# zju3dv/BoxDreamer

Measured on AMD Instinct MI355X. Metric: poses/s/GPU (5-ref, 224×224, bf16); heatmap max-abs err vs CPU ref, higher is better.
Workload: dtype f16 + e4m3 corrections (BETR q, k columns: f16)

## Files before the change

### boxdreamer_amd/csrc/gemm_f16c8.hip

```cpp
#include "gemm_common.h"

#ifdef BD_GEMM_PROBE
extern "C" int bd_gemm_f16c8_probe_set(void* buf) {
    return (int)hipMemcpyToSymbol(HIP_SYMBOL(bd_probe_buf), &buf, sizeof(buf));
}
#endif

namespace {

template <int NSTAGE, int EP, int OUTK, bool GELU, int WM = 4, int WN = 2, int NPW = 4, bool LNF = false, bool SK = false>
__global__ __launch_bounds__((WM * WN + NPW) * 64, (WM * WN + NPW) <= 4 ? 2 : 1) void gemm_kernel_pc_f16c8(const bd_gemm_args p) {
    constexpr int MI = 2, NI = 3, NCW = WM * WN;
    constexpr int TBM = WM * MI * 32, TBN = WN * NI * 32, BK = 32;
    constexpr int A0 = TBM * 64, W0 = TBN * 64, A1 = TBM * 32, W1 = TBN * 64;
    constexpr int OFF_W0 = A0, OFF_A1 = A0 + W0, OFF_W1 = A0 + W0 + A1, STAGE = A0 + W0 + A1 + W1;
    constexpr int SR = 16, SCRATCH = NCW * SR * NI * 32 * 4, S2 = SCRATCH > STAGE ? SCRATCH : STAGE;
    static_assert(SCRATCH <= STAGE, "the epilogue scratch overlays stage 2");
    constexpr int GA0 = TBM / 16, GW0 = TBN / 16, GA1 = TBM / 32, GW1 = TBN / 16;
    constexpr int IA0 = (GA0 + NPW - 1) / NPW, IW0 = (GW0 + NPW - 1) / NPW, IA1 = (GA1 + NPW - 1) / NPW, IW1 = (GW1 + NPW - 1) / NPW;
    static_assert(GA0 % NPW == 0 && GW0 % NPW == 0 && GA1 % NPW == 0 && GW1 % NPW == 0, "every producer wave issues the same number of pieces (counted vmcnt)");
    constexpr int PIECES = IA0 + IW0 + IA1 + IW1;
    constexpr int WAIT_ONE_SLAB = (PIECES & 15) | ((PIECES >> 4) << 14) | 0x70 | 0xF00;
    constexpr int AUX_COLP = 2 * STAGE + S2, AUX_RMS = AUX_COLP + 4096, AUX_ROWS = AUX_RMS + 2048, AUX_BYTES = EP == 0 ? 0 : (LNF ? 10240 : 6144);
    static_assert(!LNF || (EP != 0 && NPW * 64 >= TBM && NSTAGE == 3), "LayerNorm fold: one producer lane per tile row");
    static_assert(!SK || ((EP == 3 || EP == 4 || EP == 5) && !LNF && NSTAGE == 3), "split-K: the fp32-residual epilogues, one tile per workgroup");
    __shared__ __attribute__((aligned(1024))) unsigned char lds[2 * STAGE + S2 + AUX_BYTES];

    bd_saturating_conversions();
    const int tid = threadIdx.x, lane = tid & 63;
    const int wid = __builtin_amdgcn_readfirstlane(tid >> 6);
    const int M = p.M, N = p.N;
    const int S = SK ? p.sk_split : 1;
    const int ks = SK ? ((int)blockIdx.x >> 3) % S : 0;
    const int nk_all = p.K / BK;
    const int k_lo = SK ? ks * nk_all / S : 0;
    const int nk = SK ? (ks + 1) * nk_all / S - k_lo : nk_all;
    const int tilesM = (M + TBM - 1) / TBM, tilesN = (N + TBN - 1) / TBN, nt = tilesM * tilesN;
    const int nwg = SK ? (int)gridDim.x / S : (int)gridDim.x;
    const int bid = SK ? ((int)blockIdx.x & 7) + 8 * (((int)blockIdx.x >> 3) / S) : (int)blockIdx.x, xcd = bid & 7;
    const int tq = nt >> 3, tr = nt & 7;
    const int t_begin = xcd < tr ? xcd * (tq + 1) : tr * (tq + 1) + (xcd - tr) * tq;
    const int t_end = t_begin + tq + (xcd < tr ? 1 : 0);
    const int stride = (nwg - xcd + 7) >> 3;
    constexpr int GROUP_M = 4;
    auto tile_origin = [&](int t, int& m0, int& n0) {
        const int per_group = GROUP_M * tilesN;
        const int g = t / per_group, in_g = t % per_group;
        const int gm0 = g * GROUP_M;
        const int gh = (tilesM - gm0) < GROUP_M ? (tilesM - gm0) : GROUP_M;
        m0 = (gm0 + in_g % gh) * TBM;
        n0 = (in_g / gh) * TBN;
    };
    const unsigned lds_off = lds_offset_of(lds);

    if (wid >= NCW) {
        const int pw = wid - NCW;
        const unsigned lda0 = (unsigned)(p.lda * 2), ldw0 = (unsigned)(p.ldw * 2), lda1 = (unsigned)p.lda, ldw1 = (unsigned)(p.ldw * 2);
        unsigned oA0[IA0], oW0[IW0], oA1[IA1], oW1[IW1];
#pragma unroll
        for (int i = 0; i < IA0; ++i) { const int row = (pw + NPW * i) * 16 + lane / 4; oA0[i] = row * lda0 + swz_chunk<4>(row, lane % 4) * 16; }
#pragma unroll
        for (int i = 0; i < IW0; ++i) { const int row = (pw + NPW * i) * 16 + lane / 4; oW0[i] = row * ldw0 + swz_chunk<4>(row, lane % 4) * 16; }
#pragma unroll
        for (int i = 0; i < IA1; ++i) { const int row = (pw + NPW * i) * 32 + lane / 2; oA1[i] = row * lda1 + swz_chunk<2>(row, lane % 2) * 16; }
#pragma unroll
        for (int i = 0; i < IW1; ++i) { const int row = (pw + NPW * i) * 16 + lane / 4; oW1[i] = row * ldw1 + swz_chunk<4>(row, lane % 4) * 16; }
        const unsigned char* pA0 = (const unsigned char*)p.A;
        const unsigned char* pW0 = (const unsigned char*)p.W;
        const unsigned char* pA1 = pA0 + p.a_plane * 2;
        const unsigned char* pW1 = pW0 + p.w_plane * 2;
        auto issue = [&](int stage, int m0, int n0, int kt) {
            const int rows_a = (M - m0) < TBM ? (M - m0) : TBM, rows_w = (N - n0) < TBN ? (N - n0) : TBN;
            const unsigned la0 = (unsigned)(rows_a - 1) * lda0 + 48, lw0 = (unsigned)(rows_w - 1) * ldw0 + 48;
            const unsigned la1 = (unsigned)(rows_a - 1) * lda1 + 16, lw1 = (unsigned)(rows_w - 1) * ldw1 + 48;
            const unsigned st = lds_off + stage * STAGE + pw * 1024;
            const unsigned char* ba0 = pA0 + (int64_t)m0 * lda0 + (int64_t)(k_lo + kt) * 64;
            const unsigned char* bw0 = pW0 + (int64_t)n0 * ldw0 + (int64_t)(k_lo + kt) * 64;
            const unsigned char* ba1 = pA1 + (int64_t)m0 * lda1 + (int64_t)(k_lo + kt) * 32;
            const unsigned char* bw1 = pW1 + (int64_t)n0 * ldw1 + (int64_t)(k_lo + kt) * 64;
#pragma unroll
            for (int i = 0; i < IA0; ++i) glds16_s(oA0[i] < la0 ? oA0[i] : la0, ba0, st + i * (NPW * 1024));
#pragma unroll
            for (int i = 0; i < IW0; ++i) glds16_s(oW0[i] < lw0 ? oW0[i] : lw0, bw0, st + OFF_W0 + i * (NPW * 1024));
#pragma unroll
            for (int i = 0; i < IA1; ++i) glds16_s(oA1[i] < la1 ? oA1[i] : la1, ba1, st + OFF_A1 + i * (NPW * 1024));
#pragma unroll
            for (int i = 0; i < IW1; ++i) glds16_s(oW1[i] < lw1 ? oW1[i] : lw1, bw1, st + OFF_W1 + i * (NPW * 1024));
        };
        int ig = 0, ist = 0, it = t_begin + (bid >> 3), ikt = 0, im0 = 0, in0 = 0, itn = 0;
        if (it < t_end) tile_origin(it, im0, in0);
        if constexpr (EP == 2) {
            if (pw == 1) {
                const unsigned off = (unsigned)lane * 16 < 368u ? (unsigned)lane * 16 : 368u;
                glds16_s(off, (const unsigned char*)p.rms_wq, lds_off + AUX_RMS);
                glds16_s(off, (const unsigned char*)p.rms_wk, lds_off + AUX_RMS + 1024);
            }
        }
        int lnt = 0;
        auto issue_next = [&]() {
            if (it >= t_end) return;
            if constexpr (EP != 0) {
                if (ikt == 0) {
                    if (pw == 0 && p.bias) {
                        const unsigned off = (unsigned)lane * 16 < (unsigned)(TBN * 4 - 16) ? (unsigned)lane * 16 : (unsigned)(TBN * 4 - 16);
                        glds16_s(off, (const unsigned char*)(p.bias + in0), lds_off + AUX_COLP + (itn & 1) * 2048);
                    }
                    if constexpr (LNF) {
                        if (pw == 1 % NPW) {
                            const unsigned off = (unsigned)lane * 16 < (unsigned)(TBN * 4 - 16) ? (unsigned)lane * 16 : (unsigned)(TBN * 4 - 16);
                            glds16_s(off, (const unsigned char*)(p.ln_colsum + in0), lds_off + AUX_COLP + (itn & 1) * 2048 + 1024);
                        }
                        if (pw * 64 + lane < TBM) {
                            int row = im0 + pw * 64 + lane;
                            row = row < M ? row : M - 1;
                            const f32x4* sp = (const f32x4*)(p.ln_stats_in + (int64_t)row * 16);
                            const f32x4 lnst[4] = {sp[0], sp[1], sp[2], sp[3]};
                            *(float2*)(lds + AUX_ROWS + (lnt & 1) * 2048 + (pw * 64 + lane) * 8) = ln_rows_combine(lnst, p.ln_eps);
                        }
                        ++lnt;
                        asm volatile("s_waitcnt lgkmcnt(0)" ::: "memory");
                    }
                    ++itn;
                }
            }
            issue(ist, im0, in0, ikt);
            ++ig;
            ist = ist + 1 == NSTAGE ? 0 : ist + 1;
            if (++ikt == nk) {
                ikt = 0;
                it += stride;
                if (it < t_end) tile_origin(it, im0, in0);
            }
        };
        auto wait_landed = [&](int slabs) {
            if (slabs <= 0) asm volatile("s_waitcnt vmcnt(0)" ::: "memory");
            else { __builtin_amdgcn_s_waitcnt(WAIT_ONE_SLAB); asm volatile("" ::: "memory"); }
        };
#ifdef BD_GEMM_PROBE
        unsigned probe_ts = 0;
#endif
#pragma unroll
        for (int i = 0; i < NSTAGE - 1; ++i) issue_next();
        int g = 0;
        for (int t = t_begin + (bid >> 3); t < t_end; t += stride) {
            for (int kt = 0; kt < nk; ++kt) {
                BD_PROBE_IF(g < 20, g * 3 + 2)
                wait_landed(ig - g - 1);
                BD_PROBE_IF(g < 20, g * 3)
                pc_barrier();
                BD_PROBE_IF(g < 20, g * 3 + 1)
                if (ig <= g + NSTAGE - 1) issue_next();
                ++g;
            }
            pc_barrier();
        }
#ifdef BD_GEMM_PROBE
        if (bd_probe_buf && blockIdx.x < 1024) bd_probe_buf[((size_t)blockIdx.x * 16 + wid) * 64 + lane] = probe_ts;
#endif
        return;
    }

    const int wm = wid / WN, wn = wid % WN;
    const int lrow = lane & 31, lhalf = lane >> 5;
    const int scale_a = 127, scale_w = 127 - (p.w_qexp + BD_F16C8_D);
    int g_st = 0;
#ifdef BD_GEMM_PROBE
    unsigned probe_ts = 0;
    int g = 0;
#endif
    BD_PROBE(58) BD_PROBE_RT(56)
    int ti = 0;
    f32x16 acc[MI][NI];
    const bool secondary = SK && ks != S - 1;
    if constexpr (EP != 0) {
        int m0, n0;
        tile_origin(t_begin + (bid >> 3), m0, n0);
        if (secondary) {
#pragma unroll
            for (int i = 0; i < MI; ++i)
#pragma unroll
                for (int j = 0; j < NI; ++j)
#pragma unroll
                    for (int r = 0; r < 16; ++r) acc[i][j][r] = 0.f;
        } else {
            acc_init<MI, NI>(p, acc, m0 + wm * (MI * 32), n0 + wn * (NI * 32), lane);
        }
    }
    for (int t = t_begin + (bid >> 3); t < t_end; t += stride, ++ti) {
        int m0, n0;
        tile_origin(t, m0, n0);
        if constexpr (EP == 0) acc_init<MI, NI>(p, acc, m0 + wm * (MI * 32), n0 + wn * (NI * 32), lane);
        for (int kt = 0; kt < nk; ++kt) {
            BD_PROBE_IF(g < 20, g * 3)
            pc_barrier();
            BD_PROBE_IF(g < 20, g * 3 + 1)
#ifdef BD_GEMM_PROBE
            ++g;
#endif
            const unsigned char* base = lds + g_st * STAGE;
            g_st = g_st + 1 == NSTAGE ? 0 : g_st + 1;
            f16x8 ah[2][MI], wh[2][NI];
            u128 al[MI];
            i32x8 w8[NI];
#define LD16(dst, ptr, row, ks) dst = __builtin_bit_cast(f16x8, *(const u128*)((ptr) + (row) * 64 + (swz_chunk<4>((row), (ks) * 2 + lhalf) << 4)));
#define LDLO(dst, ptr, row) dst = *(const u128*)((ptr) + (row) * 32 + (swz_chunk<2>((row), lhalf) << 4));
#define LDW8(dst, ptr, row)                                                                                    \
            {                                                                                                     \
                const u128 lo_ = *(const u128*)((ptr) + (row) * 64 + (swz_chunk<4>((row), 2 * lhalf) << 4));        \
                const u128 hi_ = *(const u128*)((ptr) + (row) * 64 + (swz_chunk<4>((row), 2 * lhalf + 1) << 4));    \
                dst = (i32x8){(int)lo_[0], (int)lo_[1], (int)lo_[2], (int)lo_[3], (int)hi_[0], (int)hi_[1], (int)hi_[2], (int)hi_[3]}; \
            }
#define Q8P(f, a, b) ((h2_){f[a], f[b]})
#define Q8H(d0, d1, f)                                                                                        \
            {                                                                                                     \
                typedef _Float16 h2_ __attribute__((ext_vector_type(2)));                                         \
                typedef short s2_ __attribute__((ext_vector_type(2)));                                            \
                s2_ a_ = {0, 0}, b_ = {0, 0};                                                                     \
                a_ = __builtin_amdgcn_cvt_scalef32_pk_fp8_f16(a_, Q8P(f, 0, 1), 1.0f, false);                     \
                a_ = __builtin_amdgcn_cvt_scalef32_pk_fp8_f16(a_, Q8P(f, 2, 3), 1.0f, true);                      \
                b_ = __builtin_amdgcn_cvt_scalef32_pk_fp8_f16(b_, Q8P(f, 4, 5), 1.0f, false);                     \
                b_ = __builtin_amdgcn_cvt_scalef32_pk_fp8_f16(b_, Q8P(f, 6, 7), 1.0f, true);                      \
                d0 = __builtin_bit_cast(unsigned, a_);                                                            \
                d1 = __builtin_bit_cast(unsigned, b_);                                                            \
            }
#pragma unroll
            for (int j = 0; j < NI; ++j) LD16(wh[0][j], base + OFF_W0, wn * (NI * 32) + j * 32 + lrow, 0)
#pragma unroll
            for (int i = 0; i < MI; ++i) LD16(ah[0][i], base, wm * (MI * 32) + i * 32 + lrow, 0)
            __builtin_amdgcn_sched_barrier(0);
            constexpr int NMM = MI * NI;
            static_assert(MI == 2 && NI == 3, "the interleave below is written for 2 x 3 MFMA tiles per wave");
            unsigned qd[MI][4];
#pragma unroll
            for (int q = 0; q < NMM; ++q) {
                const int i = q % MI, j = q / MI;
                acc[i][j] = __builtin_amdgcn_mfma_f32_32x32x16_f16(ah[0][i], wh[0][j], acc[i][j], 0, 0, 0);
                if (q < MI) LD16(ah[1][q], base, wm * (MI * 32) + q * 32 + lrow, 1)
                else if (q < MI + NI) LD16(wh[1][q - MI], base + OFF_W0, wn * (NI * 32) + (q - MI) * 32 + lrow, 1)
                if (q == 3) Q8H(qd[0][0], qd[0][1], ah[0][0])
                if (q == 4) Q8H(qd[1][0], qd[1][1], ah[0][1])
                __builtin_amdgcn_sched_barrier(0);
            }
#pragma unroll
            for (int q = 0; q < NMM; ++q) {
                const int i = q % MI, j = q / MI;
                acc[i][j] = __builtin_amdgcn_mfma_f32_32x32x16_f16(ah[1][i], wh[1][j], acc[i][j], 0, 0, 0);
                if (q < MI) LDLO(al[q], base + OFF_A1, wm * (MI * 32) + q * 32 + lrow)
                if (q == 2) LDW8(w8[0], base + OFF_W1, wn * (NI * 32) + lrow)
                if (q == 4) LDW8(w8[1], base + OFF_W1, wn * (NI * 32) + 32 + lrow)
                if (q == 2) Q8H(qd[0][2], qd[0][3], ah[1][0])
                if (q == 3) Q8H(qd[1][2], qd[1][3], ah[1][1])
                __builtin_amdgcn_sched_barrier(0);
            }
#pragma unroll
            for (int q = 0; q < NMM; ++q) {
                const int i = q % MI, j = q / MI;
                const i32x8 a8 = {(int)al[i][0], (int)al[i][1], (int)al[i][2], (int)al[i][3], (int)qd[i][0], (int)qd[i][1], (int)qd[i][2], (int)qd[i][3]};
                acc[i][j] = __builtin_amdgcn_mfma_scale_f32_32x32x64_f8f6f4(a8, w8[j], acc[i][j], 0, 0, 0, scale_a, 0, scale_w);
                if (q == 0) LDW8(w8[2], base + OFF_W1, wn * (NI * 32) + 64 + lrow)
                __builtin_amdgcn_sched_barrier(0);
            }
#undef LDW8
#undef LD16
#undef LDLO
#undef Q8H
#undef Q8P
        }
        BD_PROBE_IF(g == nk, 60)
        pc_barrier();
        BD_PROBE_IF(g == nk, 61)
        if constexpr (SK) {
            int* const flags = (int*)p.sk_ws;
            f32x4* const parts = (f32x4*)((unsigned char*)p.sk_ws + BD_SPLITK_FLAG_BYTES);
            if (secondary) {
                const int idx = (t * 3 + ks) * NCW + wid;
                f32x4* dst = parts + (size_t)idx * (MI * NI * 4 * 64) + lane;
#pragma unroll
                for (int i = 0; i < MI; ++i)
#pragma unroll
                    for (int j = 0; j < NI; ++j)
#pragma unroll
                        for (int q = 0; q < 4; ++q) {
                            const f32x4 v = {acc[i][j][4 * q], acc[i][j][4 * q + 1], acc[i][j][4 * q + 2], acc[i][j][4 * q + 3]};
                            asm volatile("global_store_dwordx4 %0, %1, off sc1" : : "v"(dst + ((i * NI + j) * 4 + q) * 64), "v"(v) : "memory");
                        }
                asm volatile("s_waitcnt vmcnt(0)" ::: "memory");
                if (lane == 0) __hip_atomic_store(flags + idx, 1, __ATOMIC_RELAXED, __HIP_MEMORY_SCOPE_AGENT);
                return;
            }
            for (int sk = 0; sk < S - 1; ++sk) {
                const int idx = (t * 3 + sk) * NCW + wid;
                for (int spin = 0; spin < (1 << 24) && __hip_atomic_load(flags + idx, __ATOMIC_RELAXED, __HIP_MEMORY_SCOPE_AGENT) == 0; ++spin)
                    __builtin_amdgcn_s_sleep(1);
                asm volatile("" ::: "memory");
                if (lane == 0) __hip_atomic_store(flags + idx, 0, __ATOMIC_RELAXED, __HIP_MEMORY_SCOPE_AGENT);
                const f32x4* src = parts + (size_t)idx * (MI * NI * 4 * 64) + lane;
                f32x4 v[MI * NI * 4];
#pragma unroll
                for (int u = 0; u < MI * NI * 4; ++u)
                    asm volatile("global_load_dwordx4 %0, %1, off sc1" : "=v"(v[u]) : "v"(src + u * 64) : "memory");
                static_assert(MI * NI == 6, "24 register quads named below");
                asm volatile("s_waitcnt vmcnt(0)" : "+v"(v[0]), "+v"(v[1]), "+v"(v[2]), "+v"(v[3]), "+v"(v[4]), "+v"(v[5]), "+v"(v[6]), "+v"(v[7]),
                             "+v"(v[8]), "+v"(v[9]), "+v"(v[10]), "+v"(v[11]), "+v"(v[12]), "+v"(v[13]), "+v"(v[14]), "+v"(v[15]),
                             "+v"(v[16]), "+v"(v[17]), "+v"(v[18]), "+v"(v[19]), "+v"(v[20]), "+v"(v[21]), "+v"(v[22]), "+v"(v[23]) : : "memory");
#pragma unroll
                for (int i = 0; i < MI; ++i)
#pragma unroll
                    for (int j = 0; j < NI; ++j)
#pragma unroll
                        for (int q = 0; q < 4; ++q)
#pragma unroll
                            for (int e = 0; e < 4; ++e) acc[i][j][4 * q + e] += v[(i * NI + j) * 4 + q][e];
            }
        }
        unsigned char* scratch = lds + 2 * STAGE + wid * (SR * NI * 32 * 4);
        if constexpr (EP == 0) {
            gemm_epilogue_lds<f16c8, 2, MI, NI, SR, true>(p, acc, scratch, m0 + wm * (MI * 32), n0 + wn * (NI * 32), lane);
        } else {
            const bool has_next = t + stride < t_end;
            int nm0 = 0, nn0 = 0;
            if (has_next) tile_origin(t + stride, nm0, nn0);
            pc_epilogue<f16c8, 2, EP, OUTK, GELU, 2, LNF>(p, acc, (float*)scratch, (float*)scratch + 8 * 96, (const float*)(lds + AUX_COLP + (ti & 1) * 2048),
                                                 (const float*)(lds + AUX_COLP + ((ti + 1) & 1) * 2048), (const float*)(lds + AUX_RMS), wn * (NI * 32), m0 + wm * (MI * 32), n0 + wn * (NI * 32),
                                                 lane, has_next, nm0 + wm * (MI * 32), nn0 + wn * (NI * 32),
                                                 (const float*)(lds + (LNF ? AUX_ROWS : 0) + (ti & 1) * 2048), wm * (MI * 32));
        }
        BD_PROBE_IF(g == nk, 62)
    }
    BD_PROBE(59) BD_PROBE_RT(57)
#ifdef BD_GEMM_PROBE
    if (bd_probe_buf && blockIdx.x < 1024) bd_probe_buf[((size_t)blockIdx.x * 16 + wid) * 64 + lane] = probe_ts;
#endif
}

}

int& bd_concurrent_launches() {
    static thread_local int n = 1;
    return n;
}

static int f16c8_epilogue_kind(const bd_gemm_args& a, int& outk, bool& gelu) {
    int ep = 0;
    outk = a.out_f32;
    gelu = a.act == BD_ACT_GELU;
    if (!a.addtab && a.rpg_in <= 0 && !a.wscale && a.N % 192 == 0 && a.K >= 128 && !(a.bias && ((uintptr_t)a.bias & 15))) {
        if (a.out_f32 == OUT_F32) ep = (gelu || a.rms_wq) ? 0 : 3;
        else if (!a.resid && (outk == OUT_OPERAND || outk == OUT_F16 || outk == OUT_BF16X2)) ep = a.rms_wq ? (gelu ? 0 : 2) : 1;
    }
    if (ep == 1 && gelu && outk != OUT_OPERAND) ep = 0;
    return ep;
}

bool bd_f16c8_takes_ln_fold(const bd_gemm_args& a) {
    int outk = 0;
    bool gelu = false;
    const int ep = f16c8_epilogue_kind(a, outk, gelu);
    const bool s3 = (a.K / 32) % 3 == 0;
    if (!s3 || !wide_epilogue_ok(a, 2)) return false;
    if (ln_fold_producer(a)) {
        if (!ln_fold_producer_ok(a)) return false;
        const bool base = !a.addtab && a.rpg_in <= 0 && !a.wscale && a.N % 192 == 0 && a.K >= 128 && !(a.bias && ((uintptr_t)a.bias & 15)) &&
                          !gelu && !a.rms_wq;
        if (!base || (!a.ln_resid_in_op && ep != 3)) return false;
    }
    if (ln_fold_consumer(a)) {
        if (!ln_fold_consumer_ok(a)) return false;
        const bool form = (ep == 1 && gelu && outk == OUT_OPERAND) || (ep == 1 && !gelu && (outk == OUT_F16 || outk == OUT_BF16X2)) ||
                          (ep == 2 && outk == OUT_F16);
        if (!form) return false;
    }
    return true;
}

static int f16c8_split_k(const bd_gemm_args& a, int ep, bool r5, bool lnp, bool s3, int cus) {
    (void)lnp;
    if (!a.sk_ws || ((uintptr_t)a.sk_ws & 255) || !s3 || a.N % 96 != 0 || !bd_gemm_splitk_flag_bytes(a.M, a.N) || !(ep == 3 || r5)) return 1;
    const int t96 = ((a.M + 127) / 128) * (a.N / 96), nk = a.K / 32;
    const int slots = cus / (bd_concurrent_launches() > 0 ? bd_concurrent_launches() : 1);
    int sk = a.sk_split;
    if (sk <= 0) {
        sk = 1;
        for (int c = 4; c >= 2; --c)
            if (t96 * c <= slots && nk / c >= 6) { sk = c; break; }
    }
    if (sk < 2 || sk > 4 || nk / sk < 1) return 1;
    return sk;
}

extern "C" size_t bd_gemm_splitk_flag_bytes(int M, int N) {
    if (M <= 0 || N <= 0 || N % 96 != 0 || M > BD_SPLITK_MAX_ROWS) return 0;
    const size_t t96 = (size_t)((M + 127) / 128) * (size_t)(N / 96);
    return t96 * 3 * 2 * 4 <= BD_SPLITK_FLAG_BYTES ? BD_SPLITK_FLAG_BYTES : 0;
}
extern "C" size_t bd_gemm_splitk_workspace_bytes(int M, int N) {
    const size_t fb = bd_gemm_splitk_flag_bytes(M, N);
    if (!fb) return 0;
    const size_t t96 = (size_t)((M + 127) / 128) * (size_t)(N / 96);
    return fb + t96 * 3 * 2 * (size_t)(64 * 96 * 4);
}

int bd_launch_gemm_f16c8(const bd_gemm_args& a, hipStream_t s) {
    if (!wide_epilogue_ok(a, 2) || 256 * a.lda * 2 >= ((int64_t)1 << 31) || 256 * a.ldw * 2 >= ((int64_t)1 << 31)) return BD_ERR_ALIGN;
    if ((a.K % 32) || (a.lda % 32) || (a.ldw % 32)) return BD_ERR_SHAPE;
    if (a.out_f32 == OUT_OPERAND && (a.ldo % 32)) return BD_ERR_SHAPE;
    if (a.w_qexp + BD_F16C8_D < -100 || a.w_qexp + BD_F16C8_D > 120) return BD_ERR_SHAPE;
    if (a.rms_wq && !rms_geometry_ok(a)) return BD_ERR_SHAPE;
    const bool lnp = ln_fold_producer(a), lnc = ln_fold_consumer(a);
    if ((lnp || lnc) && !bd_f16c8_takes_ln_fold(a)) return BD_ERR_SHAPE;
    const int slot = bd_trace_open(s, 0, a.M, a.N, a.K);
    const int cus = cu_count();
    const int tiles = ((a.M + 255) / 256) * ((a.N + 191) / 192);
    int outk = 0;
    bool gelu = false;
    const int ep = f16c8_epilogue_kind(a, outk, gelu);
    const bool s3 = (a.K / 32) % 3 == 0;
    const int tiles_small = ((a.M + 127) / 128) * ((a.N + 191) / 192);
    const bool small = s3 && ep != 0 && 2 * tiles * bd_concurrent_launches() <= cus;
    const bool small0 = ep == 0 && 2 * tiles * bd_concurrent_launches() <= cus;
    const dim3 g0(tiles_small < cus ? tiles_small : cus);
    const int grid = small ? (tiles_small < cus ? tiles_small : cus) : (tiles < cus ? tiles : cus);
    const dim3 g(grid), b(small ? 512 : 768);
#define BD_C8_LAUNCH(EP_, OUTK_, GELU_)                                                                     \
    { if (small) hipLaunchKernelGGL((gemm_kernel_pc_f16c8<3, EP_, OUTK_, GELU_, 2, 2, 4>), g, b, 0, s, a);     \
      else if (s3) hipLaunchKernelGGL((gemm_kernel_pc_f16c8<3, EP_, OUTK_, GELU_>), g, b, 0, s, a);            \
      else hipLaunchKernelGGL((gemm_kernel_pc_f16c8<2, EP_, OUTK_, GELU_>), g, b, 0, s, a); }
#define BD_C8_LAUNCH_LN(EP_, OUTK_, GELU_, LNF_)                                                                        \
    { if (small) hipLaunchKernelGGL((gemm_kernel_pc_f16c8<3, EP_, OUTK_, GELU_, 2, 2, 4, LNF_>), g, b, 0, s, a);         \
      else hipLaunchKernelGGL((gemm_kernel_pc_f16c8<3, EP_, OUTK_, GELU_, 4, 2, 4, LNF_>), g, b, 0, s, a); }
    const bool r5 = lnp && a.ln_resid_in_op;
    const bool fc2_96 = (ep == 3 || r5) && small && a.K >= 2048 && a.N % 96 == 0 && 4 * tiles * bd_concurrent_launches() <= cus;
    const int sk = f16c8_split_k(a, ep, r5, lnp, s3, cus);
    if (sk > 1) {
        bd_gemm_args b2 = a;
        b2.sk_split = sk;
        const int t96 = ((a.M + 127) / 128) * (a.N / 96);
        const dim3 gs(((t96 + 7) / 8) * 8 * sk), bs(256);
        if (r5 && a.out_f32 == OUT_F32) hipLaunchKernelGGL((gemm_kernel_pc_f16c8<3, 5, OUT_F32, false, 2, 1, 2, false, true>), gs, bs, 0, s, b2);
        else if (r5) hipLaunchKernelGGL((gemm_kernel_pc_f16c8<3, 5, OUT_OPERAND, false, 2, 1, 2, false, true>), gs, bs, 0, s, b2);
        else if (lnp) hipLaunchKernelGGL((gemm_kernel_pc_f16c8<3, 4, OUT_F32, false, 2, 1, 2, false, true>), gs, bs, 0, s, b2);
        else hipLaunchKernelGGL((gemm_kernel_pc_f16c8<3, 3, OUT_F32, false, 2, 1, 2, false, true>), gs, bs, 0, s, b2);
        bd_trace_close(s, slot);
        BD_CHECK_LAUNCH();
        return BD_OK;
    }
    if (r5 && fc2_96 && a.out_f32 == OUT_F32)
        hipLaunchKernelGGL((gemm_kernel_pc_f16c8<3, 5, OUT_F32, false, 2, 1, 2>), dim3(((a.M + 127) / 128) * (a.N / 96)), dim3(256), 0, s, a);
    else if (r5 && fc2_96)
        hipLaunchKernelGGL((gemm_kernel_pc_f16c8<3, 5, OUT_OPERAND, false, 2, 1, 2>), dim3(((a.M + 127) / 128) * (a.N / 96)), dim3(256), 0, s, a);
    else if (r5 && a.out_f32 == OUT_F32) BD_C8_LAUNCH_LN(5, OUT_F32, false, false)
    else if (r5) BD_C8_LAUNCH_LN(5, OUT_OPERAND, false, false)
    else if (lnp && fc2_96)
        hipLaunchKernelGGL((gemm_kernel_pc_f16c8<3, 4, OUT_F32, false, 2, 1, 2>), dim3(((a.M + 127) / 128) * (a.N / 96)), dim3(256), 0, s, a);
    else if (lnp) BD_C8_LAUNCH_LN(4, OUT_F32, false, false)
    else if (lnc && ep == 1 && gelu) BD_C8_LAUNCH_LN(1, OUT_OPERAND, true, true)
    else if (lnc && ep == 1 && outk == OUT_F16) BD_C8_LAUNCH_LN(1, OUT_F16, false, true)
    else if (lnc && ep == 1) BD_C8_LAUNCH_LN(1, OUT_BF16X2, false, true)
    else if (lnc) BD_C8_LAUNCH_LN(2, OUT_F16, false, true)
    else if (fc2_96)
        hipLaunchKernelGGL((gemm_kernel_pc_f16c8<3, 3, OUT_F32, false, 2, 1, 2>), dim3(((a.M + 127) / 128) * (a.N / 96)), dim3(256), 0, s, a);
    else if (ep == 3) BD_C8_LAUNCH(3, OUT_F32, false)
    else if (ep == 2 && outk == OUT_OPERAND) BD_C8_LAUNCH(2, OUT_OPERAND, false)
    else if (ep == 2 && outk == OUT_F16) BD_C8_LAUNCH(2, OUT_F16, false)
    else if (ep == 2) BD_C8_LAUNCH(2, OUT_BF16X2, false)
    else if (ep == 1 && gelu) BD_C8_LAUNCH(1, OUT_OPERAND, true)
    else if (ep == 1 && outk == OUT_OPERAND) BD_C8_LAUNCH(1, OUT_OPERAND, false)
    else if (ep == 1 && outk == OUT_F16) BD_C8_LAUNCH(1, OUT_F16, false)
    else if (ep == 1) BD_C8_LAUNCH(1, OUT_BF16X2, false)
    else if (small0 && s3) hipLaunchKernelGGL((gemm_kernel_pc_f16c8<3, 0, OUT_OPERAND, false, 2, 2, 4>), g0, dim3(512), 0, s, a);
    else if (small0) hipLaunchKernelGGL((gemm_kernel_pc_f16c8<2, 0, OUT_OPERAND, false, 2, 2, 4>), g0, dim3(512), 0, s, a);
    else if (s3) hipLaunchKernelGGL((gemm_kernel_pc_f16c8<3, 0, OUT_OPERAND, false>), g, b, 0, s, a);
    else hipLaunchKernelGGL((gemm_kernel_pc_f16c8<2, 0, OUT_OPERAND, false>), g, b, 0, s, a);
#undef BD_C8_LAUNCH
#undef BD_C8_LAUNCH_LN
    bd_trace_close(s, slot);
    BD_CHECK_LAUNCH();
    return BD_OK;
}
```

Before: 784.2.

## Use planar per-operand LDS layout with compile-time stage slabs and precomputed fragment addresses

New measurement: 792.1, median of 6. 1.01x the previous value.

```diff
diff --git a/boxdreamer_amd/csrc/gemm_f16c8.hip b/boxdreamer_amd/csrc/gemm_f16c8.hip
--- a/boxdreamer_amd/csrc/gemm_f16c8.hip
+++ b/boxdreamer_amd/csrc/gemm_f16c8.hip
@@ -13,9 +13,12 @@
     constexpr int MI = 2, NI = 3, NCW = WM * WN;
     constexpr int TBM = WM * MI * 32, TBN = WN * NI * 32, BK = 32;
     constexpr int A0 = TBM * 64, W0 = TBN * 64, A1 = TBM * 32, W1 = TBN * 64;
-    constexpr int OFF_W0 = A0, OFF_A1 = A0 + W0, OFF_W1 = A0 + W0 + A1, STAGE = A0 + W0 + A1 + W1;
-    constexpr int SR = 16, SCRATCH = NCW * SR * NI * 32 * 4, S2 = SCRATCH > STAGE ? SCRATCH : STAGE;
-    static_assert(SCRATCH <= STAGE, "the epilogue scratch overlays stage 2");
+    constexpr int STAGE = A0 + W0 + A1 + W1;
+    constexpr int PL_A0 = 0, PL_A1 = NSTAGE * A0, PL_W0 = NSTAGE * (A0 + A1), PL_W1 = PL_W0 + NSTAGE * W0;
+    static_assert((NSTAGE - 1) * A0 + (MI - 1) * 2048 + 16 <= 65536 && (NSTAGE - 1) * W0 + (NI - 1) * 2048 + 16 <= 65536, "stage + fragment fit a DS immediate");
+    constexpr int SR = 16, WSCR = SR * NI * 32 * 4, SCRATCH = NCW * WSCR, S2 = SCRATCH > STAGE ? SCRATCH : STAGE;
+    constexpr int NSA = (A0 + A1) / WSCR < NCW ? (A0 + A1) / WSCR : NCW;
+    static_assert(SCRATCH <= STAGE && (NCW - NSA) * WSCR <= W0 + W1, "the epilogue scratch overlays stage 2");
     constexpr int GA0 = TBM / 16, GW0 = TBN / 16, GA1 = TBM / 32, GW1 = TBN / 16;
     constexpr int IA0 = (GA0 + NPW - 1) / NPW, IW0 = (GW0 + NPW - 1) / NPW, IA1 = (GA1 + NPW - 1) / NPW, IW1 = (GW1 + NPW - 1) / NPW;
     static_assert(GA0 % NPW == 0 && GW0 % NPW == 0 && GA1 % NPW == 0 && GW1 % NPW == 0, "every producer wave issues the same number of pieces (counted vmcnt)");
@@ -73,19 +76,21 @@
             const int rows_a = (M - m0) < TBM ? (M - m0) : TBM, rows_w = (N - n0) < TBN ? (N - n0) : TBN;
             const unsigned la0 = (unsigned)(rows_a - 1) * lda0 + 48, lw0 = (unsigned)(rows_w - 1) * ldw0 + 48;
             const unsigned la1 = (unsigned)(rows_a - 1) * lda1 + 16, lw1 = (unsigned)(rows_w - 1) * ldw1 + 48;
-            const unsigned st = lds_off + stage * STAGE + pw * 1024;
+            const unsigned st = lds_off + pw * 1024;
+            const unsigned sa0 = st + PL_A0 + stage * A0, sw0 = st + PL_W0 + stage * W0;
+            const unsigned sa1 = st + PL_A1 + (NSTAGE - 1 - stage) * A1, sw1 = st + PL_W1 + (NSTAGE - 1 - stage) * W1;
             const unsigned char* ba0 = pA0 + (int64_t)m0 * lda0 + (int64_t)(k_lo + kt) * 64;
             const unsigned char* bw0 = pW0 + (int64_t)n0 * ldw0 + (int64_t)(k_lo + kt) * 64;
             const unsigned char* ba1 = pA1 + (int64_t)m0 * lda1 + (int64_t)(k_lo + kt) * 32;
             const unsigned char* bw1 = pW1 + (int64_t)n0 * ldw1 + (int64_t)(k_lo + kt) * 64;
 #pragma unroll
-            for (int i = 0; i < IA0; ++i) glds16_s(oA0[i] < la0 ? oA0[i] : la0, ba0, st + i * (NPW * 1024));
-#pragma unroll
-            for (int i = 0; i < IW0; ++i) glds16_s(oW0[i] < lw0 ? oW0[i] : lw0, bw0, st + OFF_W0 + i * (NPW * 1024));
-#pragma unroll
-            for (int i = 0; i < IA1; ++i) glds16_s(oA1[i] < la1 ? oA1[i] : la1, ba1, st + OFF_A1 + i * (NPW * 1024));
-#pragma unroll
-            for (int i = 0; i < IW1; ++i) glds16_s(oW1[i] < lw1 ? oW1[i] : lw1, bw1, st + OFF_W1 + i * (NPW * 1024));
+            for (int i = 0; i < IA0; ++i) glds16_s(oA0[i] < la0 ? oA0[i] : la0, ba0, sa0 + i * (NPW * 1024));
+#pragma unroll
+            for (int i = 0; i < IW0; ++i) glds16_s(oW0[i] < lw0 ? oW0[i] : lw0, bw0, sw0 + i * (NPW * 1024));
+#pragma unroll
+            for (int i = 0; i < IA1; ++i) glds16_s(oA1[i] < la1 ? oA1[i] : la1, ba1, sa1 + i * (NPW * 1024));
+#pragma unroll
+            for (int i = 0; i < IW1; ++i) glds16_s(oW1[i] < lw1 ? oW1[i] : lw1, bw1, sw1 + i * (NPW * 1024));
         };
         int ig = 0, ist = 0, it = t_begin + (bid >> 3), ikt = 0, im0 = 0, in0 = 0, itn = 0;
         if (it < t_end) tile_origin(it, im0, in0);
@@ -164,6 +169,18 @@
     const int lrow = lane & 31, lhalf = lane >> 5;
     const int scale_a = 127, scale_w = 127 - (p.w_qexp + BD_F16C8_D);
     int g_st = 0;
+    unsigned fa0[2], fw0[2], fa1, fw1[2];
+    {
+        const int ra = wm * (MI * 32) + lrow, rw = wn * (NI * 32) + lrow;
+#pragma unroll
+        for (int k = 0; k < 2; ++k) {
+            fa0[k] = PL_A0 + ra * 64 + (swz_chunk<4>(ra, k * 2 + lhalf) << 4);
+            fw0[k] = PL_W0 + rw * 64 + (swz_chunk<4>(rw, k * 2 + lhalf) << 4);
+            fw1[k] = PL_W1 + rw * 64 + (swz_chunk<4>(rw, 2 * lhalf + k) << 4);
+        }
+        fa1 = PL_A1 + ra * 32 + (swz_chunk<2>(ra, lhalf) << 4);
+        asm volatile("" : "+v"(fa0[0]), "+v"(fa0[1]), "+v"(fw0[0]), "+v"(fw0[1]), "+v"(fa1), "+v"(fw1[0]), "+v"(fw1[1]));
+    }
 #ifdef BD_GEMM_PROBE
     unsigned probe_ts = 0;
     int g = 0;
@@ -190,24 +207,28 @@
         int m0, n0;
         tile_origin(t, m0, n0);
         if constexpr (EP == 0) acc_init<MI, NI>(p, acc, m0 + wm * (MI * 32), n0 + wn * (NI * 32), lane);
-        for (int kt = 0; kt < nk; ++kt) {
+        int sc_a = scale_a, sc_w = scale_w;
+        unsigned qd[MI][4] = {};
+        asm volatile("" : "+v"(sc_a), "+v"(sc_w));
+        auto slab = [&](auto st_) {
+            constexpr int ST = decltype(st_)::value;
+            constexpr int SA0 = ST * A0, SW0 = ST * W0, SA1 = (NSTAGE - 1 - ST) * A1, SW1 = (NSTAGE - 1 - ST) * W1;
             BD_PROBE_IF(g < 20, g * 3)
             pc_barrier();
             BD_PROBE_IF(g < 20, g * 3 + 1)
 #ifdef BD_GEMM_PROBE
             ++g;
 #endif
-            const unsigned char* base = lds + g_st * STAGE;
-            g_st = g_st + 1 == NSTAGE ? 0 : g_st + 1;
             f16x8 ah[2][MI], wh[2][NI];
             u128 al[MI];
             i32x8 w8[NI];
-#define LD16(dst, ptr, row, ks) dst = __builtin_bit_cast(f16x8, *(const u128*)((ptr) + (row) * 64 + (swz_chunk<4>((row), (ks) * 2 + lhalf) << 4)));
-#define LDLO(dst, ptr, row) dst = *(const u128*)((ptr) + (row) * 32 + (swz_chunk<2>((row), lhalf) << 4));
-#define LDW8(dst, ptr, row)                                                                                    \
+#define LD16A(dst, f, ks) dst = __builtin_bit_cast(f16x8, *(const u128*)(lds + fa0[ks] + (SA0 + (f) * 2048)));
+#define LD16W(dst, f, ks) dst = __builtin_bit_cast(f16x8, *(const u128*)(lds + fw0[ks] + (SW0 + (f) * 2048)));
+#define LDLO(dst, f) dst = *(const u128*)(lds + fa1 + (SA1 + (f) * 1024));
+#define LDW8(dst, f)                                                                                           \
             {                                                                                                     \
-                const u128 lo_ = *(const u128*)((ptr) + (row) * 64 + (swz_chunk<4>((row), 2 * lhalf) << 4));        \
-                const u128 hi_ = *(const u128*)((ptr) + (row) * 64 + (swz_chunk<4>((row), 2 * lhalf + 1) << 4));    \
+                const u128 lo_ = *(const u128*)(lds + fw1[0] + (SW1 + (f) * 2048));                               \
+                const u128 hi_ = *(const u128*)(lds + fw1[1] + (SW1 + (f) * 2048));                               \
                 dst = (i32x8){(int)lo_[0], (int)lo_[1], (int)lo_[2], (int)lo_[3], (int)hi_[0], (int)hi_[1], (int)hi_[2], (int)hi_[3]}; \
             }
 #define Q8P(f, a, b) ((h2_){f[a], f[b]})
@@ -215,7 +236,7 @@
             {                                                                                                     \
                 typedef _Float16 h2_ __attribute__((ext_vector_type(2)));                                         \
                 typedef short s2_ __attribute__((ext_vector_type(2)));                                            \
-                s2_ a_ = {0, 0}, b_ = {0, 0};                                                                     \
+                s2_ a_ = __builtin_bit_cast(s2_, d0), b_ = __builtin_bit_cast(s2_, d1);        \
                 a_ = __builtin_amdgcn_cvt_scalef32_pk_fp8_f16(a_, Q8P(f, 0, 1), 1.0f, false);                     \
                 a_ = __builtin_amdgcn_cvt_scalef32_pk_fp8_f16(a_, Q8P(f, 2, 3), 1.0f, true);                      \
                 b_ = __builtin_amdgcn_cvt_scalef32_pk_fp8_f16(b_, Q8P(f, 4, 5), 1.0f, false);                     \
@@ -224,19 +245,18 @@
                 d1 = __builtin_bit_cast(unsigned, b_);                                                            \
             }
 #pragma unroll
-            for (int j = 0; j < NI; ++j) LD16(wh[0][j], base + OFF_W0, wn * (NI * 32) + j * 32 + lrow, 0)
-#pragma unroll
-            for (int i = 0; i < MI; ++i) LD16(ah[0][i], base, wm * (MI * 32) + i * 32 + lrow, 0)
+            for (int j = 0; j < NI; ++j) LD16W(wh[0][j], j, 0)
+#pragma unroll
+            for (int i = 0; i < MI; ++i) LD16A(ah[0][i], i, 0)
             __builtin_amdgcn_sched_barrier(0);
             constexpr int NMM = MI * NI;
             static_assert(MI == 2 && NI == 3, "the interleave below is written for 2 x 3 MFMA tiles per wave");
-            unsigned qd[MI][4];
 #pragma unroll
             for (int q = 0; q < NMM; ++q) {
                 const int i = q % MI, j = q / MI;
                 acc[i][j] = __builtin_amdgcn_mfma_f32_32x32x16_f16(ah[0][i], wh[0][j], acc[i][j], 0, 0, 0);
-                if (q < MI) LD16(ah[1][q], base, wm * (MI * 32) + q * 32 + lrow, 1)
-                else if (q < MI + NI) LD16(wh[1][q - MI], base + OFF_W0, wn * (NI * 32) + (q - MI) * 32 + lrow, 1)
+                if (q < MI) LD16A(ah[1][q], q, 1)
+                else if (q < MI + NI) LD16W(wh[1][q - MI], q - MI, 1)
                 if (q == 3) Q8H(qd[0][0], qd[0][1], ah[0][0])
                 if (q == 4) Q8H(qd[1][0], qd[1][1], ah[0][1])
                 __builtin_amdgcn_sched_barrier(0);
@@ -245,9 +265,9 @@
             for (int q = 0; q < NMM; ++q) {
                 const int i = q % MI, j = q / MI;
                 acc[i][j] = __builtin_amdgcn_mfma_f32_32x32x16_f16(ah[1][i], wh[1][j], acc[i][j], 0, 0, 0);
-                if (q < MI) LDLO(al[q], base + OFF_A1, wm * (MI * 32) + q * 32 + lrow)
-                if (q == 2) LDW8(w8[0], base + OFF_W1, wn * (NI * 32) + lrow)
-                if (q == 4) LDW8(w8[1], base + OFF_W1, wn * (NI * 32) + 32 + lrow)
+                if (q < MI) LDLO(al[q], q)
+                if (q == 2) LDW8(w8[0], 0)
+                if (q == 4) LDW8(w8[1], 1)
                 if (q == 2) Q8H(qd[0][2], qd[0][3], ah[1][0])
                 if (q == 3) Q8H(qd[1][2], qd[1][3], ah[1][1])
                 __builtin_amdgcn_sched_barrier(0);
@@ -256,15 +276,33 @@
             for (int q = 0; q < NMM; ++q) {
                 const int i = q % MI, j = q / MI;
                 const i32x8 a8 = {(int)al[i][0], (int)al[i][1], (int)al[i][2], (int)al[i][3], (int)qd[i][0], (int)qd[i][1], (int)qd[i][2], (int)qd[i][3]};
-                acc[i][j] = __builtin_amdgcn_mfma_scale_f32_32x32x64_f8f6f4(a8, w8[j], acc[i][j], 0, 0, 0, scale_a, 0, scale_w);
-                if (q == 0) LDW8(w8[2], base + OFF_W1, wn * (NI * 32) + 64 + lrow)
+                acc[i][j] = __builtin_amdgcn_mfma_scale_f32_32x32x64_f8f6f4(a8, w8[j], acc[i][j], 0, 0, 0, sc_a, 0, sc_w);
+                if (q == 0) LDW8(w8[2], 2)
                 __builtin_amdgcn_sched_barrier(0);
             }
 #undef LDW8
-#undef LD16
+#undef LD16A
+#undef LD16W
 #undef LDLO
 #undef Q8H
 #undef Q8P
+        };
+        {
+            using std::integral_constant;
+            int left = nk;
+            if constexpr (NSTAGE == 3) {
+                if (g_st == 1 && left > 0) { slab(integral_constant<int, 1>{}); g_st = 2; --left; }
+            }
+            if (g_st == NSTAGE - 1 && left > 0) { slab(integral_constant<int, NSTAGE - 1>{}); g_st = 0; --left; }
+            for (; left >= NSTAGE; left -= NSTAGE) {
+                slab(integral_constant<int, 0>{});
+                slab(integral_constant<int, 1>{});
+                if constexpr (NSTAGE == 3) slab(integral_constant<int, 2>{});
+            }
+            if (left > 0) { slab(integral_constant<int, 0>{}); g_st = 1; --left; }
+            if constexpr (NSTAGE == 3) {
+                if (left > 0) { slab(integral_constant<int, 1>{}); g_st = 2; }
+            }
         }
         BD_PROBE_IF(g == nk, 60)
         pc_barrier();
@@ -313,7 +351,8 @@
                             for (int e = 0; e < 4; ++e) acc[i][j][4 * q + e] += v[(i * NI + j) * 4 + q][e];
             }
         }
-        unsigned char* scratch = lds + 2 * STAGE + wid * (SR * NI * 32 * 4);
+        unsigned char* scratch = NSTAGE != 3 ? lds + 2 * STAGE + wid * WSCR
+                                 : wid < NSA ? lds + PL_A0 + 2 * A0 + wid * WSCR : lds + PL_W0 + 2 * W0 + (wid - NSA) * WSCR;
         if constexpr (EP == 0) {
             gemm_epilogue_lds<f16c8, 2, MI, NI, SR, true>(p, acc, scratch, m0 + wm * (MI * 32), n0 + wn * (NI * 32), lane);
         } else {
```
